# PaddleCV-SIG/MedicalSeg

Hardware: AMD Instinct MI355X
Metric: 3D-voxels/sec fwd+bwd, VNet 128^3 fp32 (higher is better)
Workload: dtype f32

## Files before the change

### medicalseg_amd/csrc/msk_common.h

```cpp
#pragma once
#include <hip/hip_runtime.h>
#include <hip/hip_ext.h>

#include <cstdint>
#include <cstdio>
#include <cstring>
#include <map>
#include <set>
#include <string>
#include <utility>
#include <vector>

#include "msegk.h"

struct msk_prof_entry {
  double total_ms = 0.0;
  long calls = 0;
};

struct msk_pending_event {
  hipEvent_t a, b;
  const char* tag;
};

// ... 34 lines not shown
  int wgrad_chunk = -1;
  char prof_prefix[48] = {0};
  long wgrad_async_max_m = 0;
  float* scalar_ring = nullptr;
  int scalar_next = 0;
  long scalar_served = 0;
  float* scalar_ring_side = nullptr;
  int scalar_next_side = 0;
  long scalar_served_side = 0;
  int wbf_tpb = 0;
  void* wpack = nullptr;
  int wbf_pack_cache = 1;
  void* spack = nullptr;
  int wbf_pack_lds = 1;
  int wbf_bpf = 1;
  int wbf_ks_blocks = 2;
  int noop_after_merge = 0;
  int wgrad_c1_wpc = 2;
  int eager_tail_main = 1;
  int prof_paused = 0;
  int prof_attach = 1;
  int small_pack_cache = 1;
  int wbf_prepack = 1;
  int ks_legacy = 0;
  int wgrad_fork = 1;
  int wbf_fused_bl = 2;
  int wbf_fuse = 1;
  int conv_split = 2;
  int bwd_fuse = -1;
  int foldn_wgs = 0;
// ... 172 lines not shown
```

### medicalseg_amd/csrc/msk_conv_wbf.hip

```cpp
#include <type_traits>
#include "msk_wbf.h"
#ifndef WBF_TIN_SYNC
#define WBF_TIN_SYNC 1
#endif

#ifndef WBF_PROBE
#define WBF_PROBE 0
#endif
typedef _Float16 f16x8 __attribute__((ext_vector_type(8)));
typedef _Float16 f16x2 __attribute__((ext_vector_type(2)));

namespace {

constexpr int nxi_of(int K) { return K == 5 ? 8 : 6; }

__device__ __forceinline__ void split3_one(float x, unsigned short& hi, unsigned short& mid, unsigned short& lo) {
  hi = __builtin_bit_cast(unsigned short, (__bf16)x);
  const float r = x - __uint_as_float((unsigned)hi << 16);
  mid = __builtin_bit_cast(unsigned short, (__bf16)r);
  const float r2 = r - __uint_as_float((unsigned)mid << 16);
  lo = __builtin_bit_cast(unsigned short, (__bf16)r2);
}
__device__ __forceinline__ unsigned pack_f16_pair(float a, float b) {
  f32x2 v = {a, b};
// ... 633 lines not shown
    else if (r < 28) { a = 1; b = r - 16; }
    else { a = 1; b = r - 28; }
  } else if (TH == 8) {
    if (r < 4) { a = 0; b = r; }
    else if (r < 12) { a = 1; b = r - 4; }
    else if (r < 16) { a = 0; b = r - 8; }
    else if (r < 20) { a = 3; b = r - 16; }
    else if (r < 28) { a = 2; b = r - 20; }
    else { a = 3; b = r - 24; }
  } else {
    a = r / TH;
    b = r % TH;
  }
}

template <int MR, int WM, int WN, int TD, int TH, int K, int NP, int BPF = 1>
__global__ void __launch_bounds__(WM * WN * 64)
wbf_gemm_k(GemmArgs a) {
  static_assert((WM * WN == 4 || WM * WN == 2) && WM * MR * 32 == TD * TH, "tile shape");
  constexpr int NT = WM * WN * 64;
  constexpr int NXI = nxi_of(K), T2 = K * K, PADK = (K - 1) / 2;
  constexpr int HDt = TD + K - 1, HPt = TH + K - 1, NSLOT = HDt * HPt, NPL = 2 * NP, NIT = NPL * NSLOT, ROUNDS = (NIT + NT - 1) / NT;
  __shared__ uint4 lds[ROUNDS * NT];

  const int tid = threadIdx.x;
  const int wave = __builtin_amdgcn_readfirstlane(tid >> 6), lane = tid & 63, li = lane & 31, lh = lane >> 5;
  const int wm = wave / WN, wn = wave % WN;

#pragma unroll 1
  for (int rep = 0; rep < a.tpb; ++rep) {
  int b = blockIdx.x + rep * gridDim.x;
  if (b >= a.nblk) break;
  if (rep > 0) __syncthreads();
  const int xi = b % NXI;
  b /= NXI;
  const int grp = b % a.ngrp;
  b /= a.ngrp;
// ... 13 lines not shown
    if (it >= NIT) it = 0;
    const int pk = it / NSLOT, slot = it - pk * NSLOT;
    const int row = slot / HPt, col = slot - row * HPt;
    voff[r] = (unsigned)(pk * a.v_plane + ((long)row * a.HP + col) * 16);
  }
  const char* vtile = a.V + (long)xi * a.v_xi + ((long)(n * a.T + t) * a.KC) * NPL * a.v_plane +
                      ((long)(tdi * TD + 2 - PADK) * a.HP + thi * TH + 2 - PADK) * 16;
  const __amdgpu_buffer_rsrc_t vres = __builtin_amdgcn_make_buffer_rsrc((void*)vtile, 0, 0xFFFFFFF0u, 0x00020000);
  const __amdgpu_buffer_rsrc_t ures =
      __builtin_amdgcn_make_buffer_rsrc((void*)(a.U + (long)xi * a.u_xi), 0, 0xFFFFFFF0u, 0x00020000);
  const unsigned ulane = (unsigned)(lh * a.CN + (grp * WN + wn) * 32 + li) * 16u;
  const unsigned ustep = (unsigned)a.CN * 32u;
  const unsigned uchunk = (unsigned)NP * ustep;
  const unsigned utap = (unsigned)a.KC * uchunk;

  int arow[MR];
#pragma unroll
  for (int mr = 0; mr < MR; ++mr) {
    int fa, fb;
    frag_pos<TH>(li, fa, fb);
    arow[mr] = lh * NSLOT + ((wm * MR + mr) * (32 / TH) + fa) * HPt + fb;
  }

  f32x16 acc[MR];
#pragma unroll
  for (int mr = 0; mr < MR; ++mr)
#pragma unroll
    for (int j = 0; j < 16; ++j) acc[mr][j] = 0.f;

  const int kc0 = ks * a.kc_per;
  const int kc1 = min(a.KC, kc0 + a.kc_per);
  for (int kc = kc0; kc < kc1; ++kc) {
    __syncthreads();
    const unsigned vsoff = (unsigned)(kc * NPL * a.v_plane);
#pragma unroll
    for (int r = 0; r < ROUNDS; ++r)
      __builtin_amdgcn_raw_ptr_buffer_load_lds(vres, (__attribute__((address_space(3))) void*)(lds + r * NT + wave * 64), 16,
                                               (int)voff[r], (int)vsoff, 0, 0);
    const unsigned ukc = (unsigned)kc * uchunk;
    constexpr int BR = BPF + 1;
    uint4 bq[BR][NP];
#pragma unroll
    for (int t0 = 0; t0 < BPF && t0 < T2; ++t0)
#pragma unroll
      for (int p = 0; p < NP; ++p) bq[t0][p] = buf_load16(ures, ulane, (unsigned)t0 * utap + ukc + p * ustep);
    asm volatile("s_waitcnt vmcnt(0)" ::: "memory");
// ... 56 lines not shown
      __builtin_amdgcn_sched_barrier(0);
    }
  }

  const int co = (grp * WN + wn) * 32 + li;
  float* mbase = a.M + ((long)ks * NXI + xi) * a.m_xi + ((long)(n * a.T + t) * a.LD) * a.LH * a.CN + co;
#pragma unroll
  for (int mr = 0; mr < MR; ++mr) {
#pragma unroll
    for (int j = 0; j < 16; ++j) {
      int fa, fb;
      frag_pos<TH>((j & 3) + 8 * (j >> 2) + 4 * lh, fa, fb);
      const int d = tdi * TD + (wm * MR + mr) * (32 / TH) + fa, h = thi * TH + fb;
      if (d < a.LD && h < a.LH) mbase[((long)d * a.LH + h) * a.CN] = acc[mr][j];
    }
  }
  }
}

struct FusedArgs {
  GemmArgs g;
  float* dst;
  int dld;
  long dvn;
  int dvd, dvh, dvw;
  const float* bias;
  const float* prelu;
  int accumulate;
  const float* in_amax;
  const float* w_amax;
// ... 26 lines not shown
  const int last = K == 5 ? 7 : 5;
  c0 = xi == last ? 0.f : 1.f;
  if (xi == 0) { c1 = c2 = c3 = 0.f; return; }
  if (xi == last) { c1 = c2 = 0.f; c3 = 1.f; return; }
  const float sg = (xi & 1) ? 1.f : -1.f;
  const int pr = (xi - 1) >> 1;
  const float p = pr == 0 ? 1.f : (pr == 1 ? 2.f : 0.5f);
  c1 = sg * p;
  c2 = p * p;
  c3 = sg * p * p * p;
}

#ifndef WBF_FUSED_BPF
#define WBF_FUSED_BPF 3
#endif
template <int MR, int WM, int WN, int TD, int TH, int K, int NP, bool STATS, int BPF = (NP == 2 ? WBF_FUSED_BPF : 1), int BL = 0>
__global__ void __launch_bounds__(WM * WN * 64, 2)
wbf_gemm_fused_k(FusedArgs f) {
  static_assert(WM * WN == 4 && WM * MR * 32 == TD * TH, "tile shape");
  const GemmArgs& a = f.g;
  constexpr int NT = WM * WN * 64;
  constexpr int NXI = nxi_of(K), T2 = K * K, PADK = (K - 1) / 2;
  constexpr int HDt = TD + K - 1, HPt = TH + K - 1, NSLOT = HDt * HPt, NPL = 2 * NP, NIT = NPL * NSLOT, ROUNDS = (NIT + NT - 1) / NT;
  constexpr int NBF = T2 * NP;
  constexpr int BROUNDS = (NBF + WM * WN - 1) / (WM * WN);
  static_assert(BL == 0 || NIT % 64 == 0, "weights through LDS: wave-granular tile");
  static_assert(BL != 1 || WN == 1, "B through LDS, whole stage: one column fragment");
  constexpr int PH = WN == 1 ? 4 : 5;
  constexpr int PQ_T[6] = {0, T2 * 1 / PH, T2 * 2 / PH, T2 * 3 / PH, PH > 4 ? T2 * 4 / PH : T2, T2};
  constexpr int PQ_FR = (T2 - PQ_T[PH - 1]) * NP * WN;
  constexpr int PQ_SLOT = PQ_FR * 64;
  static_assert(BL != 2 || (NP == 2 && WM * WN == 4 && WN <= 2 && PQ_T[1] * NP * WN >= 4), "pipelined form: fp16 x 2 pieces, four wavefronts");
  __shared__ uint4 lds[BL == 2 ? 2 * NIT + 2 * PQ_SLOT : (BL ? NIT + NBF * 64 : ROUNDS * NT)];

// ... 30 lines not shown
  int arow[MR];
#pragma unroll
  for (int mr = 0; mr < MR; ++mr) {
    int fa, fb;
    frag_pos<TH>(li, fa, fb);
    arow[mr] = lh * NSLOT + ((wm * MR + mr) * (32 / TH) + fa) * HPt + fb;
  }

  f32x16 yo[4][MR];
#pragma unroll
  for (int i = 0; i < 4; ++i)
#pragma unroll
    for (int mr = 0; mr < MR; ++mr)
#pragma unroll
      for (int j = 0; j < 16; ++j) yo[i][mr][j] = 0.f;

  if constexpr (BL == 2) {
    const unsigned lds0 = (unsigned)(unsigned long)(__attribute__((address_space(3))) void*)lds;
    const int NS = NXI * a.KC;
    const unsigned voff_last = (ROUNDS - 1) * NT + wave * 64 < NIT ? voff[ROUNDS - 1] : voff[ROUNDS - 2];
    const int r_last = (ROUNDS - 1) * NT + wave * 64 < NIT ? ROUNDS - 1 : ROUNDS - 2;
    auto rsrc_of = [](const char* p_) {
      const unsigned long pa = (unsigned long)p_;
      i32x4 r_ = {(int)__builtin_amdgcn_readfirstlane((unsigned)pa), (int)(__builtin_amdgcn_readfirstlane((unsigned)(pa >> 32)) & 0xffffu),
                  (int)0xFFFFFFF0u, 0x00020000};
      return r_;
    };
    auto fill_tile = [&](int s_) {
      const int xi_ = s_ / a.KC, kc_ = s_ - xi_ * a.KC;
      const i32x4 vr = rsrc_of(vtile0 + (long)xi_ * a.v_xi);
// ... 53 lines not shown
#pragma unroll
            for (int p = 0; p < NP; ++p) aq[nx][mr][p] = ap[p * 2 * NSLOT];
          }
        }
        __builtin_amdgcn_sched_barrier(0);
        const uint4 bdown = wbf_hi_down(bq[cur][0]);
#pragma unroll
        for (int mr = 0; mr < MR; ++mr) WBF_MFMA_H(acc[mr], aq[cur][mr][NP - 1], bdown);
#pragma unroll
        for (int mr = 0; mr < MR; ++mr) WBF_MFMA_H(acc[mr], aq[cur][mr][0], bq[cur][NP - 1]);
#pragma unroll
        for (int mr = 0; mr < MR; ++mr) WBF_MFMA_H(acc[mr], aq[cur][mr][0], bq[cur][0]);
        __builtin_amdgcn_sched_barrier(0);
      }
    };
    fill_weights(0, std::integral_constant<int, 0>{});
    fill_tile(0);
#pragma unroll 1
    for (int s_ = 0; s_ < NS; ++s_) {
      const int xi = s_ / a.KC, kc = s_ - xi * a.KC;
      if (kc == 0) {
#pragma unroll
        for (int mr = 0; mr < MR; ++mr)
#pragma unroll
          for (int j = 0; j < 16; ++j) acc[mr][j] = 0.f;
      }
#pragma unroll
      for (int mr = 0; mr < MR; ++mr) abase[mr] = arow[mr] + (s_ & 1) * NIT;
      run_phase(s_, std::integral_constant<int, 0>{});
      run_phase(s_, std::integral_constant<int, 1>{});
      run_phase(s_, std::integral_constant<int, 2>{});
      run_phase(s_, std::integral_constant<int, 3>{});
// ... 1 lines not shown
      if (kc == a.KC - 1) {
        float c0, c1, c2, c3;
        at_column<K>(xi, c0, c1, c2, c3);
#pragma unroll
        for (int mr = 0; mr < MR; ++mr)
#pragma unroll
          for (int j = 0; j < 16; ++j) {
            const float m = acc[mr][j];
            yo[0][mr][j] = fmaf(c0, m, yo[0][mr][j]);
            yo[1][mr][j] = fmaf(c1, m, yo[1][mr][j]);
            yo[2][mr][j] = fmaf(c2, m, yo[2][mr][j]);
            yo[3][mr][j] = fmaf(c3, m, yo[3][mr][j]);
          }
      }
    }
    __syncthreads();
  } else {
#pragma unroll 1
  for (int xi = 0; xi < NXI; ++xi) {
    const __amdgpu_buffer_rsrc_t vres =
        __builtin_amdgcn_make_buffer_rsrc((void*)(vtile0 + (long)xi * a.v_xi), 0, 0xFFFFFFF0u, 0x00020000);
    const __amdgpu_buffer_rsrc_t ures =
        __builtin_amdgcn_make_buffer_rsrc((void*)(a.U + (long)xi * a.u_xi), 0, 0xFFFFFFF0u, 0x00020000);
    f32x16 acc[MR];
#pragma unroll
    for (int mr = 0; mr < MR; ++mr)
#pragma unroll
      for (int j = 0; j < 16; ++j) acc[mr][j] = 0.f;

#pragma unroll 1
// ... 158 lines not shown
    }
    float c0, c1, c2, c3;
    at_column<K>(xi, c0, c1, c2, c3);
#pragma unroll
    for (int mr = 0; mr < MR; ++mr)
#pragma unroll
      for (int j = 0; j < 16; ++j) {
        const float m = acc[mr][j];
        yo[0][mr][j] = fmaf(c0, m, yo[0][mr][j]);
        yo[1][mr][j] = fmaf(c1, m, yo[1][mr][j]);
        yo[2][mr][j] = fmaf(c2, m, yo[2][mr][j]);
        yo[3][mr][j] = fmaf(c3, m, yo[3][mr][j]);
      }
  }

  }
  const int co = wn * 32 + li;
  const float osc = f.scaled ? 1.f / (wbf_scale_of(f.in_amax) * wbf_scale_of(f.w_amax)) : 1.f;
  const float bv = f.bias ? f.bias[co] : 0.f;
  const float sl = f.prelu ? f.prelu[co] : 1.f;
  float* obase = f.dst + ((long)n * f.dvn + (long)(4 * t) * f.dvw) * f.dld + co;
  const long wst = (long)f.dvw * f.dld;
  const bool split_st = f.st_lo != nullptr;
  float* sbase = split_st ? (co < f.csplit ? f.st_lo + co : f.st_hi + (co - f.csplit)) + (((long)n * f.dvn + (long)(4 * t) * f.dvw) * f.dld >> 1) : obase;
  const long swst = split_st ? (wst >> 1) : wst;
  const long aoff = f.acc_src ? (f.acc_src - f.dst) : 0;
  const int wlim = f.LW - 4 * t;
  float sk = 0.f, s1 = 0.f, s2 = 0.f, cnt = 0.f;
#pragma unroll
  for (int mr = 0; mr < MR; ++mr) {
// ... 216 lines not shown
      __syncthreads();
    }
    if (vl == 0) {
      const int c = (t % c4n) * 4;
#pragma unroll
      for (int j = 0; j < 4; ++j) {
        float* p_ = a.stat_partial + ((long)blockIdx.x * a.CN + c + j) * 3;
        p_[0] = sh[j][t].n;
        p_[1] = sh[j][t].mean;
        p_[2] = sh[j][t].m2;
      }
    }
  }
}

template <int MR, int WM, int WN, int TD, int TH, int K, int NP>
void launch_gemm(msk_ctx* ctx, const char* tag, const GemmArgs& a, long nblk) {
  GemmArgs b = a;
  b.nblk = (int)nblk;
  int tpb = ctx->wbf_tpb > 0 ? ctx->wbf_tpb : 1;
  while (tpb > 1 && nblk / tpb < 6L * ctx->num_cu) tpb >>= 1;
  long grid = (nblk + tpb - 1) / tpb;
  grid = (grid + 7) & ~7L;
  b.tpb = (int)((nblk + grid - 1) / grid);
  const bool deep = MR == 2 && (ctx->wbf_bpf == 4 || (ctx->wbf_bpf == 0 && nblk <= 8L * ctx->num_cu));
  if constexpr (MR == 2) {
    if (deep) {
      MSK_LAUNCH_TIMED(ctx, tag, (wbf_gemm_k<MR, WM, WN, TD, TH, K, NP, 4>), dim3((unsigned)grid), dim3(WM * WN * 64), 0, b);
      return;
    }
  }
  MSK_LAUNCH_TIMED(ctx, tag, (wbf_gemm_k<MR, WM, WN, TD, TH, K, NP>), dim3((unsigned)grid), dim3(WM * WN * 64), 0, b);
}

struct Var { int id, MR, WM, WN, TD, TH; };
const Var kVars[7] = {{4, 2, 4, 1, 16, 16}, {0, 4, 4, 1, 16, 32},
                      {5, 2, 2, 2, 8, 16},  {1, 4, 2, 2, 16, 16},
                      {3, 2, 1, 4, 8, 8},   {2, 4, 1, 4, 8, 16},
                      {6, 4, 2, 1, 16, 16}};
// ... 11 lines not shown
      const Var& m2 = kVars[v0];
      const long tiles2 = (long)geo.T * ((geo.LD + m2.TD - 1) / m2.TD) * ((geo.LH + m2.TH - 1) / m2.TH);
      first = ctx->wbf_fuse == 0 || (ctx->wbf_fuse != 2 && tiles2 < (long)ctx->num_cu);
    }
    if (first) return &m4;
  }
  for (int c = v0; c < v0 + (K == 5 ? 2 : 1); ++c) {
    const Var& v = kVars[c];
    if (K == 5 && ctx->wbf_variant >= 0 && ctx->wbf_variant != v.id) continue;
    if (wbf_tile_ok(geo, v.TD, v.TH)) return &v;
  }
  return nullptr;
}

template <int K, int NP>
void launch_gemm_variant(msk_ctx* ctx, const char* tag, int variant, const GemmArgs& ga, long nblk) {
  switch (variant) {
    case 3: launch_gemm<2, 1, 4, 8, 8, K, NP>(ctx, tag, ga, nblk); break;
    case 4: launch_gemm<2, 4, 1, 16, 16, K, NP>(ctx, tag, ga, nblk); break;
    case 5: launch_gemm<2, 2, 2, 8, 16, K, NP>(ctx, tag, ga, nblk); break;
    default:
      if constexpr (K == 5) {
        if (variant == 6) launch_gemm<4, 2, 1, 16, 16, 5, NP>(ctx, tag, ga, nblk);
        else if (variant == 0) launch_gemm<4, 4, 1, 16, 32, 5, NP>(ctx, tag, ga, nblk);
        else if (variant == 1) launch_gemm<4, 2, 2, 16, 16, 5, NP>(ctx, tag, ga, nblk);
        else launch_gemm<4, 1, 4, 8, 16, 5, NP>(ctx, tag, ga, nblk);
      }
      break;
  }
}

struct WbfPackEntry {
  WbfPackDesc d{};
  int K = 0, NP = 0;
  size_t u_bytes = 0;
  bool live = false, valid = false;
  long last_use = 0;
};
struct WbfPackCache {
  static constexpr int kRows = 250;
  WbfPackEntry e[kRows];
// ... 129 lines not shown
  return free_row;
}

template <int MR, int WM, int WN, int TD, int TH, int K, int NP>
void launch_fused(msk_ctx* ctx, const char* tag, const FusedArgs& fa, bool stats, bool fork) {
  const dim3 grid((unsigned)(8 * fa.per_xcd));
  constexpr int NITc = 2 * NP * (TD + K - 1) * (TH + K - 1);
  if constexpr (WN == 2 && WM == 2 && NP == 2 && NITc % 64 == 0) {
    if (ctx->wbf_fused_bl == 2 && fa.g.CN == 64) {
      if (stats) MSK_LAUNCH_TIMED_F(ctx, tag, fork, (wbf_gemm_fused_k<MR, WM, WN, TD, TH, K, NP, true, 1, 2>), grid, dim3(WM * WN * 64), 0, fa);
      else MSK_LAUNCH_TIMED_F(ctx, tag, fork, (wbf_gemm_fused_k<MR, WM, WN, TD, TH, K, NP, false, 1, 2>), grid, dim3(WM * WN * 64), 0, fa);
      return;
    }
  }
  if constexpr (WN == 1 && NP == 2 && NITc % 64 == 0) {
    if (ctx->wbf_fused_bl == 2 && fa.g.CN == 32) {
      if (stats) MSK_LAUNCH_TIMED_F(ctx, tag, fork, (wbf_gemm_fused_k<MR, WM, WN, TD, TH, K, NP, true, 1, 2>), grid, dim3(WM * WN * 64), 0, fa);
      else MSK_LAUNCH_TIMED_F(ctx, tag, fork, (wbf_gemm_fused_k<MR, WM, WN, TD, TH, K, NP, false, 1, 2>), grid, dim3(WM * WN * 64), 0, fa);
      return;
    }
    if (ctx->wbf_fused_bl && fa.g.CN == 32) {
      if (stats) MSK_LAUNCH_TIMED_F(ctx, tag, fork, (wbf_gemm_fused_k<MR, WM, WN, TD, TH, K, NP, true, 1, 1>), grid, dim3(WM * WN * 64), 0, fa);
      else MSK_LAUNCH_TIMED_F(ctx, tag, fork, (wbf_gemm_fused_k<MR, WM, WN, TD, TH, K, NP, false, 1, 1>), grid, dim3(WM * WN * 64), 0, fa);
      return;
    }
  }
  if (stats) MSK_LAUNCH_TIMED_F(ctx, tag, fork, (wbf_gemm_fused_k<MR, WM, WN, TD, TH, K, NP, true>), grid, dim3(WM * WN * 64), 0, fa);
  else MSK_LAUNCH_TIMED_F(ctx, tag, fork, (wbf_gemm_fused_k<MR, WM, WN, TD, TH, K, NP, false>), grid, dim3(WM * WN * 64), 0, fa);
}
template <int K, int NP>
// ... 9 lines not shown
int run_pipeline(msk_ctx* ctx, const GConv& g, const float* w_canon, int A, int B, int swap, const WbfGeom& geo, const Var* bv, bool dry) {
  constexpr int NXI = nxi_of(K), NPL = 2 * NP;
  const int TD = bv->TD, TH = bv->TH, variant = bv->id;
  const int* pm = geo.perm;
  const int LD = geo.LD, LH = geo.LH, LW = geo.LW;
  const int vstr[3] = {g.DH * g.DW, g.DW, 1};
  const int tstr[3] = {K * K, K, 1};
  const int T = geo.T, KC = g.CK / 16;
  const int tiles_d = (LD + TD - 1) / TD, tiles_h = (LH + TH - 1) / TH;
  const int DP = geo.DP, HP = geo.HP;
  const int WN = bv->WN;
  const int ngrp = g.CN / (WN * 32);

  const long base_blocks = (long)NXI * ngrp * tiles_h * tiles_d * T * g.N;
  int ksplit = 1, kc_per = KC;
  if (base_blocks < 3L * ctx->num_cu && ctx->wbf_fuse != 2) {
    long want = ((long)ctx->wbf_ks_blocks * ctx->num_cu + base_blocks - 1) / base_blocks;
    if (want > KC) want = KC;
    kc_per = (int)((KC + want - 1) / want);
    ksplit = (KC + kc_per - 1) / kc_per;
  }
  const long nblk = base_blocks * ksplit;
  if (nblk > 0x7fffffffL) return 0;

  const size_t v_plane = (size_t)DP * HP * 16;
  const size_t v_xi = (size_t)g.N * T * KC * NPL * v_plane;
  const size_t m_xi = (size_t)g.N * T * LD * LH * g.CN;
  if (v_xi >= 0xFFFFFFF0ull) return 0;
  const size_t u_xi = (size_t)K * K * KC * NPL * g.CN * 16;
  if (u_xi >= 0xFFFFFFF0ull) return 0;
  if (dry) return 1;
  const bool fuse_out = ctx->wbf_fuse != 0 && ksplit == 1 && ngrp == 1 && (variant == 3 || variant == 4 || variant == 5) &&
                        NXI * u_xi <= ((size_t)3584 << 10) && (base_blocks / NXI >= 2L * ctx->num_cu || ctx->wbf_fuse == 2);
  const size_t v_bytes = (NXI * v_xi + 255) & ~(size_t)255;
// ... 64 lines not shown
        ctx->fork_recorded = true;
      }
    } else if (msk_wbf_transform(ctx, 0, K, NP, ta) != 0) {
      return -1;
    }
  }
  const bool fork_after = g.fuse && g.fuse->Y && ctx->wgrad_async && ctx->side != nullptr && ctx->wgrad_fork == 1 && ctx->fork_attach != 0;
  GemmArgs ga{};
  ga.V = V; ga.U = U; ga.M = M;
  ga.N = g.N; ga.T = T; ga.KC = KC; ga.CN = g.CN; ga.LD = LD; ga.LH = LH; ga.DP = DP; ga.HP = HP;
  ga.tiles_d = tiles_d; ga.tiles_h = tiles_h; ga.ngrp = ngrp; ga.ksplit = ksplit; ga.kc_per = kc_per;
  ga.v_xi = (long)v_xi; ga.v_plane = (long)v_plane; ga.u_xi = (long)u_xi; ga.m_xi = (long)m_xi;
  const char* tag = NP == 3 ? "wbf_gemm_k" : (NP == 2 ? "wbf_gemm_h2_k" : "wbf_gemm_f16_k");
  if (ctx->prof && ctx->prof_shapes) {
    char buf[200];
    snprintf(buf, sizeof(buf), "%s[ck=%d,cn=%d,n=%d,dhw=%dx%dx%d,k=%d,ks=%d%s]", tag, g.CK, g.CN, g.N, g.DD, g.DH, g.DW, K, ksplit,
             fuse_out ? ",fused" : "");
    tag = msk_intern_tag(ctx, buf);
  }
  if (fuse_out) {
    FusedArgs fa{};
    fa.g = ga;
    fa.g.nblk = (int)(base_blocks / NXI);
    fa.dst = g.dst; fa.dld = g.dld;
    fa.dvn = (long)g.DD * g.DH * g.DW; fa.dvd = vstr[pm[0]]; fa.dvh = vstr[pm[1]]; fa.dvw = vstr[pm[2]];
    fa.bias = g.bias; fa.prelu = g.prelu; fa.accumulate = g.accumulate;
    fa.acc_src = g.accumulate ? g.acc_src : nullptr;
    fa.in_amax = in_amax; fa.w_amax = w_amax; fa.scaled = NP != 3 ? 1 : 0;
    fa.stat_partial = SP;
    fa.per_xcd = (fa.g.nblk + 7) / 8;
    fa.LW = LW;
    if (g.dst_lo && g.dst_hi && g.dst_csplit > 0 && g.accumulate && g.dld == 2 * g.dst_csplit && g.CN == 2 * g.dst_csplit && !fuse_stats) {
// ... 10 lines not shown
          if (g.fin) {
            fn = *g.fin;
            const long o = (long)n * g.fin_stride;
            fn.save_mean += o; fn.save_invstd += o; fn.scale += o; fn.shift += o;
          }
          if (msk_bn_stats_merge(ctx, SP + (size_t)n * tps * g.CN * 3, tps, g.CN, g.stats + (size_t)n * 2 * g.CN, g.fin ? &fn : nullptr) != 0) return -1;
        }
      } else if (msk_bn_stats_merge(ctx, SP, fa.g.nblk, g.CN, g.stats, g.fin) != 0) {
        return -1;
      }
      ctx->stats_fused = true;
    }
    if (g.xform) ctx->xform_written = true;
    return 1;
  }
  launch_gemm_variant<K, NP>(ctx, tag, variant, ga, nblk);
  MSK_LAUNCH_CHECK(ctx);
  {
    ToutArgs oa{};
    oa.M = M; oa.m_xi = (long)m_xi; oa.ksplit = ksplit;
    oa.N = g.N; oa.T = T; oa.LD = LD; oa.LH = LH; oa.LW = LW; oa.CN = g.CN;
    oa.dst = g.dst; oa.dld = g.dld;
    oa.dvn = (long)g.DD * g.DH * g.DW; oa.dvd = vstr[pm[0]]; oa.dvh = vstr[pm[1]]; oa.dvw = vstr[pm[2]];
    oa.bias = g.bias; oa.prelu = g.prelu; oa.accumulate = g.accumulate;
    oa.acc_src = g.accumulate ? g.acc_src : nullptr;
    oa.stat_partial = SP;
    oa.in_amax = in_amax;
    oa.w_amax = w_amax;
    oa.scaled = NP != 3 ? 1 : 0;
    if (fuse_stats) MSK_LAUNCH_TIMED_F(ctx, "wbf_tout_k", false, (wbf_tout_k<true, K>), dim3((unsigned)tout_blocks), dim3(256), 0, oa);
    else MSK_LAUNCH_TIMED_F(ctx, "wbf_tout_k", fork_after, (wbf_tout_k<false, K>), dim3((unsigned)tout_blocks), dim3(256), 0, oa);
// ... 210 lines not shown
```

### medicalseg_amd/csrc/msk_ctx.hip

```cpp
#include <cstdlib>

#include "msk_common.h"

thread_local std::string g_msk_global_err;

int msk_fail(msk_ctx* ctx, const char* file, int line, const char* what, const char* detail) {
  char buf[1024];
  const char* base = strrchr(file, '/');
  snprintf(buf, sizeof(buf), "%s:%d: %s: %s", base ? base + 1 : file, line, what, detail ? detail : "");
  if (ctx) ctx->err = buf;
  g_msk_global_err = buf;
  return -1;
}

static void* grow(msk_ctx* ctx, void** p, size_t* cur, size_t bytes) {
  if (bytes <= *cur) return *p;
  if (*p) {
    hipStreamSynchronize(ctx->stream);
    hipFree(*p);
    *p = nullptr;
    *cur = 0;
  }
  size_t want = bytes + (bytes >> 2);
  if (hipMalloc(p, want) != hipSuccess) {
// ... 355 lines not shown
  if (len) *len = (int)s.size() + 1;
  if (buf && buflen > 0) {
    strncpy(buf, s.c_str(), buflen - 1);
    buf[buflen - 1] = 0;
  }
  return 0;
}

int msk_get_option(msk_ctx* ctx, const char* key, int* value) {
  MSK_REQUIRE(ctx, key != nullptr && value != nullptr, "msk_get_option: null argument");
  if (strcmp(key, "dp_mode") == 0) *value = ctx->dp_mode;
  else if (strcmp(key, "conv_split") == 0) *value = ctx->conv_split;
  else if (strcmp(key, "wgrad_async") == 0) *value = ctx->wgrad_async ? 1 : 0;
  else if (strcmp(key, "world") == 0) *value = ctx->world;
  else if (strcmp(key, "rank") == 0) *value = ctx->rank;
  else if (strcmp(key, "scalar_ring_served") == 0) *value = (int)(ctx->scalar_served & 0x3FFFFFFF);
  else if (strcmp(key, "scalar_ring_served_side") == 0) *value = (int)(ctx->scalar_served_side & 0x3FFFFFFF);
  else return msk_fail(ctx, __FILE__, __LINE__, "msk_get_option", "unknown key");
  return 0;
}
int msk_set_option(msk_ctx* ctx, const char* key, int value) {
  if (strcmp(key, "conv_impl") == 0) {
    ctx->conv_impl = value;
    return 0;
  }
  if (strcmp(key, "halo_tile") == 0) {
    ctx->halo_tile = value;
    return 0;
  }
  if (strcmp(key, "prof_only_halo") == 0) {
// ... 34 lines not shown
  }
  if (strcmp(key, "wbf_pad_min_voxels") == 0) {
    ctx->wbf_pad_min_voxels = value > 0 ? value : 0;
    return 0;
  }
  if (strcmp(key, "wbf_pack_cache") == 0) {
    ctx->wbf_pack_cache = value;
    return 0;
  }
  if (strcmp(key, "wbf_pack_lds") == 0) {
    ctx->wbf_pack_lds = value;
    return 0;
  }
  if (strcmp(key, "wbf_bpf") == 0) {
    ctx->wbf_bpf = value;
    return 0;
  }
  if (strcmp(key, "wbf_ks_blocks") == 0) {
    ctx->wbf_ks_blocks = value > 0 ? value : 2;
    return 0;
  }
  if (strcmp(key, "wgrad_c1_wpc") == 0) {
    ctx->wgrad_c1_wpc = value < 1 ? 1 : value;
    return 0;
  }
  if (strcmp(key, "eager_tail_main") == 0) {
    ctx->eager_tail_main = value;
    return 0;
  }
  if (strcmp(key, "fork_attach") == 0) {
// ... 172 lines not shown
```

Baseline: 252.4 million.

## Add 16x16x32 MFMA stage form for Winograd GEMM and fused kernels

Adds an alternative inner-product form to the Winograd-domain GEMM kernels that uses 16x16x32 f16 MFMA instructions instead of the 32-wide form. It processes two input-channel chunks per stage and splits output columns into two 16-wide fragments. The form is enabled by default for K=5, NP=2 shapes in both the standalone GEMM (WN>1, even KC) and the fused output kernel (CN=32, BL=2). The fused kernel also gets a matching epilogue with bias, PReLU and stats reduction. K-split chunks are rounded to even counts to match the paired stages. The aim is better MFMA throughput and data reuse. The cost is more register pressure from the extra yo16 accumulators and a new layout and epilogue path.

```diff
diff --git a/medicalseg_amd/csrc/msk_common.h b/medicalseg_amd/csrc/msk_common.h
--- a/medicalseg_amd/csrc/msk_common.h
+++ b/medicalseg_amd/csrc/msk_common.h
@@ -72,6 +72,8 @@
   void* spack = nullptr;
   int wbf_pack_lds = 1;
   int wbf_bpf = 1;
+  int wbf_fused_sh = 1;
+  int wbf_gemm_form = -1;
   int wbf_ks_blocks = 2;
   int noop_after_merge = 0;
   int wgrad_c1_wpc = 2;
diff --git a/medicalseg_amd/csrc/msk_conv_wbf.hip b/medicalseg_amd/csrc/msk_conv_wbf.hip
--- a/medicalseg_amd/csrc/msk_conv_wbf.hip
+++ b/medicalseg_amd/csrc/msk_conv_wbf.hip
@@ -671,13 +671,24 @@
   }
 }
 
-template <int MR, int WM, int WN, int TD, int TH, int K, int NP, int BPF = 1>
+template <int TH>
+__device__ __forceinline__ void subfrag_pos(int g, int r, int& d, int& h) {
+  if (TH == 8) { d = (g >> 1) * 4 + (g & 1) + 2 * (r >> 3); h = r & 7; }
+  else { d = g / (TH / 16); h = (g % (TH / 16)) * 16 + r; }
+}
+#define WBF_MFMA16_H(acc, wv, av) \
+  acc = __builtin_amdgcn_mfma_f32_16x16x32_f16(__builtin_bit_cast(f16x8, wv), __builtin_bit_cast(f16x8, av), acc, 0, 0, 0)
+
+template <int MR, int WM, int WN, int TD, int TH, int K, int NP, int BPF = 1, int SH = 32>
 __global__ void __launch_bounds__(WM * WN * 64)
 wbf_gemm_k(GemmArgs a) {
   static_assert((WM * WN == 4 || WM * WN == 2) && WM * MR * 32 == TD * TH, "tile shape");
+  static_assert(SH == 32 || (SH == 16 && NP == 2 && BPF == 1), "stage form");
+  constexpr int CPS = SH == 16 ? 2 : 1;
   constexpr int NT = WM * WN * 64;
   constexpr int NXI = nxi_of(K), T2 = K * K, PADK = (K - 1) / 2;
-  constexpr int HDt = TD + K - 1, HPt = TH + K - 1, NSLOT = HDt * HPt, NPL = 2 * NP, NIT = NPL * NSLOT, ROUNDS = (NIT + NT - 1) / NT;
+  constexpr int HDt = TD + K - 1, HPt = TH + K - 1, NSLOT = HDt * HPt, NPL = 2 * NP, NIT = CPS * NPL * NSLOT, ROUNDS = (NIT + NT - 1) / NT;
+  static_assert(SH == 32 || NSLOT % 16 == 0, "planes of the image start on a bank row (subfrag_pos)");
   __shared__ uint4 lds[ROUNDS * NT];
 
   const int tid = threadIdx.x;
@@ -721,6 +732,101 @@
   const unsigned uchunk = (unsigned)NP * ustep;
   const unsigned utap = (unsigned)a.KC * uchunk;
 
+  const int kc0 = ks * a.kc_per;
+  const int kc1 = min(a.KC, kc0 + a.kc_per);
+  if constexpr (SH == 16) {
+  constexpr int NS = 2 * MR;
+  const int l16 = lane & 15, kq = lane >> 4;
+  int arow[NS];
+#pragma unroll
+  for (int s = 0; s < NS; ++s) {
+    int dd, hh;
+    subfrag_pos<TH>(wm * NS + s, l16, dd, hh);
+    arow[s] = ((kq >> 1) * NPL + (kq & 1)) * NSLOT + dd * HPt + hh;
+  }
+  const unsigned ulane16 = (unsigned)((kq & 1) * a.CN + (grp * WN + wn) * 32 + l16) * 16u + (unsigned)(kq >> 1) * uchunk;
+  f32x4 acc[NS][2];
+#pragma unroll
+  for (int s = 0; s < NS; ++s)
+#pragma unroll
+    for (int ct = 0; ct < 2; ++ct) acc[s][ct] = f32x4{0.f, 0.f, 0.f, 0.f};
+
+  for (int kc = kc0; kc < kc1; kc += 2) {
+    __syncthreads();
+    const unsigned vsoff = (unsigned)(kc * NPL * a.v_plane);
+#pragma unroll
+    for (int r = 0; r < ROUNDS; ++r)
+      __builtin_amdgcn_raw_ptr_buffer_load_lds(vres, (__attribute__((address_space(3))) void*)(lds + r * NT + wave * 64), 16,
+                                               (int)voff[r], (int)vsoff, 0, 0);
+    const unsigned ukc = (unsigned)kc * uchunk;
+    uint4 bq[2][2][NP];
+#pragma unroll
+    for (int ct = 0; ct < 2; ++ct)
+#pragma unroll
+      for (int p = 0; p < NP; ++p) bq[0][ct][p] = buf_load16(ures, ulane16 + ct * 256u, ukc + p * ustep);
+    asm volatile("s_waitcnt vmcnt(0)" ::: "memory");
+    __syncthreads();
+
+    uint4 aq[2][MR][NP];
+    uint4 bdown[2];
+#pragma unroll
+    for (int m = 0; m < MR; ++m) {
+      const uint4* ap = lds + arow[m];
+#pragma unroll
+      for (int p = 0; p < NP; ++p) aq[0][m][p] = ap[p * 2 * NSLOT];
+    }
+#pragma unroll
+    for (int it = 0; it < 2 * T2; ++it) {
+      const int tap = it >> 1, half = it & 1, cur = it & 1, nx = cur ^ 1, bcur = tap & 1;
+      if (half == 0 && tap + 1 < T2) {
+        const unsigned ub = (unsigned)(tap + 1) * utap + ukc;
+#pragma unroll
+        for (int ct = 0; ct < 2; ++ct)
+#pragma unroll
+          for (int p = 0; p < NP; ++p) bq[bcur ^ 1][ct][p] = buf_load16(ures, ulane16 + ct * 256u, ub + p * ustep);
+      }
+      if (it + 1 < 2 * T2) {
+        const int t1 = (it + 1) >> 1, h1 = (it + 1) & 1;
+#pragma unroll
+        for (int m = 0; m < MR; ++m) {
+          const uint4* ap = lds + arow[h1 * MR + m] + (t1 / K) * HPt + (t1 % K);
+#pragma unroll
+          for (int p = 0; p < NP; ++p) aq[nx][m][p] = ap[p * 2 * NSLOT];
+        }
+      }
+      __builtin_amdgcn_sched_barrier(0);
+      if (half == 0) {
+#pragma unroll
+        for (int ct = 0; ct < 2; ++ct) bdown[ct] = wbf_hi_down(bq[bcur][ct][0]);
+      }
+#pragma unroll
+      for (int m = 0; m < MR; ++m)
+#pragma unroll
+        for (int ct = 0; ct < 2; ++ct) WBF_MFMA16_H(acc[half * MR + m][ct], bdown[ct], aq[cur][m][NP - 1]);
+#pragma unroll
+      for (int m = 0; m < MR; ++m)
+#pragma unroll
+        for (int ct = 0; ct < 2; ++ct) WBF_MFMA16_H(acc[half * MR + m][ct], bq[bcur][ct][NP - 1], aq[cur][m][0]);
+#pragma unroll
+      for (int m = 0; m < MR; ++m)
+#pragma unroll
+        for (int ct = 0; ct < 2; ++ct) WBF_MFMA16_H(acc[half * MR + m][ct], bq[bcur][ct][0], aq[cur][m][0]);
+      __builtin_amdgcn_sched_barrier(0);
+    }
+  }
+
+  float* mbase = a.M + ((long)ks * NXI + xi) * a.m_xi + ((long)(n * a.T + t) * a.LD) * a.LH * a.CN + (grp * WN + wn) * 32 + 4 * kq;
+#pragma unroll
+  for (int s = 0; s < NS; ++s) {
+    int dd, hh;
+    subfrag_pos<TH>(wm * NS + s, l16, dd, hh);
+    const int d = tdi * TD + dd, h = thi * TH + hh;
+    if (d < a.LD && h < a.LH) {
+#pragma unroll
+      for (int ct = 0; ct < 2; ++ct) *(f32x4*)(mbase + ((long)d * a.LH + h) * a.CN + ct * 16) = acc[s][ct];
+    }
+  }
+  } else {
   int arow[MR];
 #pragma unroll
   for (int mr = 0; mr < MR; ++mr) {
@@ -735,8 +841,6 @@
 #pragma unroll
     for (int j = 0; j < 16; ++j) acc[mr][j] = 0.f;
 
-  const int kc0 = ks * a.kc_per;
-  const int kc1 = min(a.KC, kc0 + a.kc_per);
   for (int kc = kc0; kc < kc1; ++kc) {
     __syncthreads();
     const unsigned vsoff = (unsigned)(kc * NPL * a.v_plane);
@@ -823,6 +927,7 @@
       const int d = tdi * TD + (wm * MR + mr) * (32 / TH) + fa, h = thi * TH + fb;
       if (d < a.LD && h < a.LH) mbase[((long)d * a.LH + h) * a.CN] = acc[mr][j];
     }
+  }
   }
   }
 }
@@ -879,10 +984,12 @@
 #ifndef WBF_FUSED_BPF
 #define WBF_FUSED_BPF 3
 #endif
-template <int MR, int WM, int WN, int TD, int TH, int K, int NP, bool STATS, int BPF = (NP == 2 ? WBF_FUSED_BPF : 1), int BL = 0>
+template <int MR, int WM, int WN, int TD, int TH, int K, int NP, bool STATS, int BPF = (NP == 2 ? WBF_FUSED_BPF : 1), int BL = 0, int SH = 32>
 __global__ void __launch_bounds__(WM * WN * 64, 2)
 wbf_gemm_fused_k(FusedArgs f) {
   static_assert(WM * WN == 4 && WM * MR * 32 == TD * TH, "tile shape");
+  static_assert(SH == 32 || (SH == 16 && BL == 2 && WN == 1 && NP == 2), "16x16x32: pipelined form, one column fragment");
+  constexpr int NS16 = 2 * MR;
   const GemmArgs& a = f.g;
   constexpr int NT = WM * WN * 64;
   constexpr int NXI = nxi_of(K), T2 = K * K, PADK = (K - 1) / 2;
@@ -943,6 +1050,14 @@
     for (int mr = 0; mr < MR; ++mr)
 #pragma unroll
       for (int j = 0; j < 16; ++j) yo[i][mr][j] = 0.f;
+  f32x4 yo16[4][NS16][2];
+#pragma unroll
+  for (int i = 0; i < 4; ++i)
+#pragma unroll
+    for (int s = 0; s < NS16; ++s)
+#pragma unroll
+      for (int ct = 0; ct < 2; ++ct) yo16[i][s][ct] = f32x4{0.f, 0.f, 0.f, 0.f};
+  const int l16 = lane & 15, kq = lane >> 4;
 
   if constexpr (BL == 2) {
     const unsigned lds0 = (unsigned)(unsigned long)(__attribute__((address_space(3))) void*)lds;
@@ -1026,8 +1141,107 @@
         __builtin_amdgcn_sched_barrier(0);
       }
     };
+    f32x4 acc16[NS16][2];
+    int arow16[NS16], abase16[NS16];
+#pragma unroll
+    for (int s = 0; s < NS16; ++s) {
+      int dd, hh;
+      subfrag_pos<TH>(wm * NS16 + s, l16, dd, hh);
+      arow16[s] = (kq & 1) * NSLOT + dd * HPt + hh;
+    }
+    auto run_phase16 = [&](int s_, auto qc) {
+      constexpr int q = decltype(qc)::value;
+      constexpr int T0 = PQ_T[q], T1 = PQ_T[q + 1], NPAIR = (T1 - T0 + 1) / 2;
+      const bool more = s_ + 1 < NS;
+      if (q == 1 && more) asm volatile("s_waitcnt vmcnt(%0)" ::"n"(ROUNDS) : "memory");
+      else asm volatile("s_waitcnt vmcnt(0)" ::: "memory");
+      __builtin_amdgcn_s_barrier();
+      asm volatile("" ::: "memory");
+      if constexpr (q < PH - 1) fill_weights(s_, std::integral_constant<int, q + 1>{});
+      else if (more) fill_weights(s_ + 1, std::integral_constant<int, 0>{});
+      if (q == 0 && more) fill_tile(s_ + 1);
+      const uint4* bl = lds + 2 * NIT + ((q + (s_ & PH & 1)) & 1) * PQ_SLOT + (kq & 1) * 32 + l16;
+      const uint4* blk = bl + (kq >> 1) * NP * 64;
+      const bool up = (kq >> 1) != 0;
+      uint4 aq[2][NP], bq[2][2][NP], bdown[2];
+      auto load_b = [&](int j, uint4 (&d_)[2][NP]) {
+        const bool full = T0 + 2 * j + 1 < T1;
+#pragma unroll
+        for (int ct = 0; ct < 2; ++ct)
+#pragma unroll
+          for (int p = 0; p < NP; ++p) {
+            if (full) {
+              d_[ct][p] = blk[(2 * j * NP + p) * 64 + ct * 16];
+            } else {
+              const uint4 v = bl[(2 * j * NP + p) * 64 + ct * 16];
+              d_[ct][p] = up ? uint4{0u, 0u, 0u, 0u} : v;
+            }
+          }
+      };
+      auto load_a = [&](int j, int sf, uint4 (&d_)[NP]) {
+        const int t0 = T0 + 2 * j, t1 = t0 + 1 < T1 ? t0 + 1 : t0;
+        const int off = up ? (t1 / K) * HPt + (t1 % K) : (t0 / K) * HPt + (t0 % K);
+        const uint4* ap = lds + abase16[sf] + off;
+#pragma unroll
+        for (int p = 0; p < NP; ++p) d_[p] = ap[p * 2 * NSLOT];
+      };
+      load_b(0, bq[0]);
+      load_a(0, 0, aq[0]);
+#pragma unroll
+      for (int it = 0; it < NS16 * NPAIR; ++it) {
+        const int j = it / NS16, sf = it % NS16, cur = it & 1, nx = cur ^ 1, bcur = j & 1;
+        if (sf == 0 && j + 1 < NPAIR) load_b(j + 1, bq[bcur ^ 1]);
+        if (it + 1 < NS16 * NPAIR) load_a((it + 1) / NS16, (it + 1) % NS16, aq[nx]);
+        __builtin_amdgcn_sched_barrier(0);
+        if (sf == 0) {
+#pragma unroll
+          for (int ct = 0; ct < 2; ++ct) bdown[ct] = wbf_hi_down(bq[bcur][ct][0]);
+        }
+#pragma unroll
+        for (int ct = 0; ct < 2; ++ct) WBF_MFMA16_H(acc16[sf][ct], aq[cur][NP - 1], bdown[ct]);
+#pragma unroll
+        for (int ct = 0; ct < 2; ++ct) WBF_MFMA16_H(acc16[sf][ct], aq[cur][0], bq[bcur][ct][NP - 1]);
+#pragma unroll
+        for (int ct = 0; ct < 2; ++ct) WBF_MFMA16_H(acc16[sf][ct], aq[cur][0], bq[bcur][ct][0]);
+        __builtin_amdgcn_sched_barrier(0);
+      }
+    };
     fill_weights(0, std::integral_constant<int, 0>{});
     fill_tile(0);
+    if constexpr (SH == 16) {
+#pragma unroll 1
+    for (int s_ = 0; s_ < NS; ++s_) {
+      const int xi = s_ / a.KC, kc = s_ - xi * a.KC;
+      if (kc == 0) {
+#pragma unroll
+        for (int s = 0; s < NS16; ++s)
+#pragma unroll
+          for (int ct = 0; ct < 2; ++ct) acc16[s][ct] = f32x4{0.f, 0.f, 0.f, 0.f};
+      }
+#pragma unroll
+      for (int s = 0; s < NS16; ++s) abase16[s] = arow16[s] + (s_ & 1) * NIT;
+      run_phase16(s_, std::integral_constant<int, 0>{});
+      run_phase16(s_, std::integral_constant<int, 1>{});
+      run_phase16(s_, std::integral_constant<int, 2>{});
+      run_phase16(s_, std::integral_constant<int, 3>{});
+      if (kc == a.KC - 1) {
+        float c0, c1, c2, c3;
+        at_column<K>(xi, c0, c1, c2, c3);
+#pragma unroll
+        for (int s = 0; s < NS16; ++s)
+#pragma unroll
+          for (int ct = 0; ct < 2; ++ct)
+#pragma unroll
+            for (int j = 0; j < 4; ++j) {
+              const float m = acc16[s][ct][j];
+              yo16[0][s][ct][j] = fmaf(c0, m, yo16[0][s][ct][j]);
+              yo16[1][s][ct][j] = fmaf(c1, m, yo16[1][s][ct][j]);
+              yo16[2][s][ct][j] = fmaf(c2, m, yo16[2][s][ct][j]);
+              yo16[3][s][ct][j] = fmaf(c3, m, yo16[3][s][ct][j]);
+            }
+      }
+    }
+    } else {
 #pragma unroll 1
     for (int s_ = 0; s_ < NS; ++s_) {
       const int xi = s_ / a.KC, kc = s_ - xi * a.KC;
@@ -1059,6 +1273,7 @@
           }
       }
     }
+    }
     __syncthreads();
   } else {
 #pragma unroll 1
@@ -1247,6 +1462,110 @@
       }
   }
 
+  }
+  if constexpr (SH == 16) {
+    const float osc = f.scaled ? 1.f / (wbf_scale_of(f.in_amax) * wbf_scale_of(f.w_amax)) : 1.f;
+    const long vox0 = ((long)n * f.dvn + (long)(4 * t) * f.dvw) * f.dld;
+    const long wst = (long)f.dvw * f.dld;
+    const bool split_st = f.st_lo != nullptr;
+    const long swst = split_st ? (wst >> 1) : wst;
+    const long aoff = f.acc_src ? (f.acc_src - f.dst) : 0;
+    const int wlim = f.LW - 4 * t;
+    WfRec rec[2];
+#pragma unroll
+    for (int ct = 0; ct < 2; ++ct) {
+      const int co = ct * 16 + l16;
+      const float bv = f.bias ? f.bias[co] : 0.f;
+      const float sl = f.prelu ? f.prelu[co] : 1.f;
+      float* obase = f.dst + vox0 + co;
+      float* sbase = split_st ? (co < f.csplit ? f.st_lo + co : f.st_hi + (co - f.csplit)) + (vox0 >> 1) : obase;
+      float sk = 0.f, s1 = 0.f, s2 = 0.f, cnt = 0.f;
+#pragma unroll
+      for (int s = 0; s < NS16; ++s) {
+        float* op[4];
+        bool ok[4];
+#pragma unroll
+        for (int jj = 0; jj < 4; ++jj) {
+          int dd, hh;
+          subfrag_pos<TH>(wm * NS16 + s, 4 * kq + jj, dd, hh);
+          const int d = tdi * TD + dd, h = thi * TH + hh;
+          ok[jj] = d < a.LD && h < a.LH;
+          op[jj] = obase + ((long)d * f.dvd + (long)h * f.dvh) * f.dld;
+        }
+        float old[4][4];
+        if (f.accumulate) {
+#pragma unroll
+          for (int jj = 0; jj < 4; ++jj)
+#pragma unroll
+            for (int i = 0; i < 4; ++i) old[jj][i] = (ok[jj] && i < wlim) ? __builtin_nontemporal_load(op[jj] + aoff + i * wst) : 0.f;
+        }
+#pragma unroll
+        for (int jj = 0; jj < 4; ++jj) {
+          if (!ok[jj]) continue;
+#pragma unroll
+          for (int i = 0; i < 4; ++i) {
+            if (i >= wlim) break;
+            float r = fmaf(yo16[i][s][ct][jj], osc, bv);
+            if (f.accumulate) r += old[jj][i];
+            if (f.prelu) r = r > 0.f ? r : sl * r;
+            if (split_st) sbase[((op[jj] - obase) >> 1) + i * swst] = r;
+            else op[jj][i * wst] = r;
+            if (STATS) {
+              if (cnt == 0.f) sk = r;
+              const float dlt = r - sk;
+              s1 += dlt;
+              s2 = fmaf(dlt, dlt, s2);
+              cnt += 1.f;
+            }
+          }
+        }
+      }
+      rec[ct] = WfRec{0.f, 0.f, 0.f};
+      if (STATS && cnt > 0.f) {
+        rec[ct].n = cnt;
+        rec[ct].mean = sk + s1 / cnt;
+        rec[ct].m2 = fmaxf(s2 - s1 * s1 / cnt, 0.f);
+      }
+    }
+    if (STATS) {
+#pragma unroll
+      for (int ct = 0; ct < 2; ++ct) {
+        WfRec w = rec[ct], o;
+        o.n = __shfl_xor(w.n, 16, 64);
+        o.mean = __shfl_xor(w.mean, 16, 64);
+        o.m2 = __shfl_xor(w.m2, 16, 64);
+        w = (kq & 1) == 0 ? wfrec_merge(w, o) : wfrec_merge(o, w);
+        o.n = __shfl_xor(w.n, 32, 64);
+        o.mean = __shfl_xor(w.mean, 32, 64);
+        o.m2 = __shfl_xor(w.m2, 32, 64);
+        rec[ct] = (kq & 2) == 0 ? wfrec_merge(w, o) : wfrec_merge(o, w);
+      }
+      __syncthreads();
+      float* sh = reinterpret_cast<float*>(lds);
+      if (kq == 0) {
+#pragma unroll
+        for (int ct = 0; ct < 2; ++ct) {
+          float* p_ = sh + (wave * 32 + ct * 16 + l16) * 3;
+          p_[0] = rec[ct].n; p_[1] = rec[ct].mean; p_[2] = rec[ct].m2;
+        }
+      }
+      __syncthreads();
+      if (wm == 0 && kq == 0) {
+#pragma unroll
+        for (int ct = 0; ct < 2; ++ct) {
+          WfRec r = rec[ct];
+#pragma unroll
+          for (int q = 1; q < WM; ++q) {
+            const float* p_ = sh + (q * 32 + ct * 16 + l16) * 3;
+            WfRec e = {p_[0], p_[1], p_[2]};
+            r = wfrec_merge(r, e);
+          }
+          float* g_ = f.stat_partial + ((long)tile_id * a.CN + ct * 16 + l16) * 3;
+          g_[0] = r.n; g_[1] = r.mean; g_[2] = r.m2;
+        }
+      }
+    }
+    return;
   }
   const int co = wn * 32 + li;
   const float osc = f.scaled ? 1.f / (wbf_scale_of(f.in_amax) * wbf_scale_of(f.w_amax)) : 1.f;
@@ -1493,8 +1812,16 @@
   }
 }
 
+template <int WN, int K, int NP>
+constexpr bool gemm_has_forms() { return K == 5 && NP == 2 && WN > 1; }
+bool gemm_pair_class(int WN, int K, int NP, int KC) { return K == 5 && NP == 2 && WN > 1 && (KC & 1) == 0; }
+int pick_gemm_form(const msk_ctx* ctx, int WN, int K, int NP, int KC) {
+  if (!gemm_pair_class(WN, K, NP, KC) || ctx->wbf_bpf != 1) return 0;
+  return ctx->wbf_gemm_form == 0 ? 0 : 2;
+}
+
 template <int MR, int WM, int WN, int TD, int TH, int K, int NP>
-void launch_gemm(msk_ctx* ctx, const char* tag, const GemmArgs& a, long nblk) {
+void launch_gemm(msk_ctx* ctx, const char* tag, const GemmArgs& a, long nblk, int form) {
   GemmArgs b = a;
   b.nblk = (int)nblk;
   int tpb = ctx->wbf_tpb > 0 ? ctx->wbf_tpb : 1;
@@ -1502,6 +1829,12 @@
   long grid = (nblk + tpb - 1) / tpb;
   grid = (grid + 7) & ~7L;
   b.tpb = (int)((nblk + grid - 1) / grid);
+  if constexpr (gemm_has_forms<WN, K, NP>()) {
+    if (form == 2) {
+      MSK_LAUNCH_TIMED(ctx, tag, (wbf_gemm_k<MR, WM, WN, TD, TH, K, NP, 1, 16>), dim3((unsigned)grid), dim3(WM * WN * 64), 0, b);
+      return;
+    }
+  }
   const bool deep = MR == 2 && (ctx->wbf_bpf == 4 || (ctx->wbf_bpf == 0 && nblk <= 8L * ctx->num_cu));
   if constexpr (MR == 2) {
     if (deep) {
@@ -1543,17 +1876,17 @@
 }
 
 template <int K, int NP>
-void launch_gemm_variant(msk_ctx* ctx, const char* tag, int variant, const GemmArgs& ga, long nblk) {
+void launch_gemm_variant(msk_ctx* ctx, const char* tag, int variant, const GemmArgs& ga, long nblk, int form) {
   switch (variant) {
-    case 3: launch_gemm<2, 1, 4, 8, 8, K, NP>(ctx, tag, ga, nblk); break;
-    case 4: launch_gemm<2, 4, 1, 16, 16, K, NP>(ctx, tag, ga, nblk); break;
-    case 5: launch_gemm<2, 2, 2, 8, 16, K, NP>(ctx, tag, ga, nblk); break;
+    case 3: launch_gemm<2, 1, 4, 8, 8, K, NP>(ctx, tag, ga, nblk, form); break;
+    case 4: launch_gemm<2, 4, 1, 16, 16, K, NP>(ctx, tag, ga, nblk, form); break;
+    case 5: launch_gemm<2, 2, 2, 8, 16, K, NP>(ctx, tag, ga, nblk, form); break;
     default:
       if constexpr (K == 5) {
-        if (variant == 6) launch_gemm<4, 2, 1, 16, 16, 5, NP>(ctx, tag, ga, nblk);
-        else if (variant == 0) launch_gemm<4, 4, 1, 16, 32, 5, NP>(ctx, tag, ga, nblk);
-        else if (variant == 1) launch_gemm<4, 2, 2, 16, 16, 5, NP>(ctx, tag, ga, nblk);
-        else launch_gemm<4, 1, 4, 8, 16, 5, NP>(ctx, tag, ga, nblk);
+        if (variant == 6) launch_gemm<4, 2, 1, 16, 16, 5, NP>(ctx, tag, ga, nblk, form);
+        else if (variant == 0) launch_gemm<4, 4, 1, 16, 32, 5, NP>(ctx, tag, ga, nblk, form);
+        else if (variant == 1) launch_gemm<4, 2, 2, 16, 16, 5, NP>(ctx, tag, ga, nblk, form);
+        else launch_gemm<4, 1, 4, 8, 16, 5, NP>(ctx, tag, ga, nblk, form);
       }
       break;
   }
@@ -1713,6 +2046,11 @@
     }
   }
   if constexpr (WN == 1 && NP == 2 && NITc % 64 == 0) {
+    if (ctx->wbf_fused_bl == 2 && fa.g.CN == 32 && ctx->wbf_fused_sh != 0) {
+      if (stats) MSK_LAUNCH_TIMED_F(ctx, tag, fork, (wbf_gemm_fused_k<MR, WM, WN, TD, TH, K, NP, true, 1, 2, 16>), grid, dim3(WM * WN * 64), 0, fa);
+      else MSK_LAUNCH_TIMED_F(ctx, tag, fork, (wbf_gemm_fused_k<MR, WM, WN, TD, TH, K, NP, false, 1, 2, 16>), grid, dim3(WM * WN * 64), 0, fa);
+      return;
+    }
     if (ctx->wbf_fused_bl == 2 && fa.g.CN == 32) {
       if (stats) MSK_LAUNCH_TIMED_F(ctx, tag, fork, (wbf_gemm_fused_k<MR, WM, WN, TD, TH, K, NP, true, 1, 2>), grid, dim3(WM * WN * 64), 0, fa);
       else MSK_LAUNCH_TIMED_F(ctx, tag, fork, (wbf_gemm_fused_k<MR, WM, WN, TD, TH, K, NP, false, 1, 2>), grid, dim3(WM * WN * 64), 0, fa);
@@ -1752,10 +2090,12 @@
 
   const long base_blocks = (long)NXI * ngrp * tiles_h * tiles_d * T * g.N;
   int ksplit = 1, kc_per = KC;
+  const int form = pick_gemm_form(ctx, WN, K, NP, KC);
   if (base_blocks < 3L * ctx->num_cu && ctx->wbf_fuse != 2) {
     long want = ((long)ctx->wbf_ks_blocks * ctx->num_cu + base_blocks - 1) / base_blocks;
     if (want > KC) want = KC;
     kc_per = (int)((KC + want - 1) / want);
+    if (gemm_pair_class(WN, K, NP, KC)) kc_per = (kc_per + 1) & ~1;
     ksplit = (KC + kc_per - 1) / kc_per;
   }
   const long nblk = base_blocks * ksplit;
@@ -1850,8 +2190,9 @@
   const char* tag = NP == 3 ? "wbf_gemm_k" : (NP == 2 ? "wbf_gemm_h2_k" : "wbf_gemm_f16_k");
   if (ctx->prof && ctx->prof_shapes) {
     char buf[200];
-    snprintf(buf, sizeof(buf), "%s[ck=%d,cn=%d,n=%d,dhw=%dx%dx%d,k=%d,ks=%d%s]", tag, g.CK, g.CN, g.N, g.DD, g.DH, g.DW, K, ksplit,
-             fuse_out ? ",fused" : "");
+    const bool sh16 = fuse_out && K == 5 && NP == 2 && variant == 4 && g.CN == 32 && ctx->wbf_fused_bl == 2 && ctx->wbf_fused_sh != 0;
+    snprintf(buf, sizeof(buf), "%s[ck=%d,cn=%d,n=%d,dhw=%dx%dx%d,k=%d,ks=%d%s%s]", tag, g.CK, g.CN, g.N, g.DD, g.DH, g.DW, K, ksplit,
+             fuse_out ? (sh16 ? ",fused,sh16" : ",fused") : "", fuse_out || form == 0 ? "" : ",form=2");
     tag = msk_intern_tag(ctx, buf);
   }
   if (fuse_out) {
@@ -1892,7 +2233,7 @@
     if (g.xform) ctx->xform_written = true;
     return 1;
   }
-  launch_gemm_variant<K, NP>(ctx, tag, variant, ga, nblk);
+  launch_gemm_variant<K, NP>(ctx, tag, variant, ga, nblk, form);
   MSK_LAUNCH_CHECK(ctx);
   {
     ToutArgs oa{};
diff --git a/medicalseg_amd/csrc/msk_ctx.hip b/medicalseg_amd/csrc/msk_ctx.hip
--- a/medicalseg_amd/csrc/msk_ctx.hip
+++ b/medicalseg_amd/csrc/msk_ctx.hip
@@ -393,6 +393,7 @@
   else if (strcmp(key, "wgrad_async") == 0) *value = ctx->wgrad_async ? 1 : 0;
   else if (strcmp(key, "world") == 0) *value = ctx->world;
   else if (strcmp(key, "rank") == 0) *value = ctx->rank;
+  else if (strcmp(key, "num_cu") == 0) *value = ctx->num_cu;
   else if (strcmp(key, "scalar_ring_served") == 0) *value = (int)(ctx->scalar_served & 0x3FFFFFFF);
   else if (strcmp(key, "scalar_ring_served_side") == 0) *value = (int)(ctx->scalar_served_side & 0x3FFFFFFF);
   else return msk_fail(ctx, __FILE__, __LINE__, "msk_get_option", "unknown key");
@@ -457,6 +458,14 @@
   }
   if (strcmp(key, "wbf_bpf") == 0) {
     ctx->wbf_bpf = value;
+    return 0;
+  }
+  if (strcmp(key, "wbf_fused_sh") == 0) {
+    ctx->wbf_fused_sh = value != 0 ? 1 : 0;
+    return 0;
+  }
+  if (strcmp(key, "wbf_gemm_form") == 0) {
+    ctx->wbf_gemm_form = value == 0 || value == 2 ? value : -1;
     return 0;
   }
   if (strcmp(key, "wbf_ks_blocks") == 0) {
```

New measurement: 257.7 million (median of 6 runs). +2.1%, better.
